# ideafisher/ssUnet-GAN

Measured on AMD Instinct MI355X. Metric: train images/sec (512^2 tiles), higher is better.
Workload: dtype f32; 1 GPU; UNet_R_SS_v2 generator + SRGAN-style discriminator, one G+D step (train_seg_gan.py:182-233), 16 x 3x512x512 tiles per GPU, fp32, Adam lr 2e-5; global_batch=16, tile=512, parallelism=dp1, dead_d_param_grads_of_g_step=computed

## Files before the change

ssunet-gan_amd/csrc/conv_wgrad4.hip:

```cpp
#include "common.h"
#include "conv_thin.h"

namespace {

struct W4Args {
  const float* wide; const float* thin; float* ws;
  int Cw, ldw, ldt, N, H, W, Cout, Cin;
  int groups, nz;
  long long units_per_z;
  int segs_per_row;
};

constexpr int SEG = 32;
constexpr int U = 8;

template <bool THIN_COUT, int KS>
__global__ __launch_bounds__(256) void wgrad4_kernel(const W4Args a) {
  constexpr int R = KS / 2, NT = KS * KS, COLS = U + KS - 1;
  const int lane = threadIdx.x & 63;
  const int wave = threadIdx.x >> 6;
  const int zb = blockIdx.x / a.groups, cg = blockIdx.x - zb * a.groups;
  const int z = zb * 4 + wave;
  const int j = lane & 3;
  const int cw = cg * 64 + lane;
  const bool cw_ok = cw < a.Cw;
  const float* tapT = THIN_COUT ? a.wide : a.thin;
  const float* fixT = THIN_COUT ? a.thin : a.wide;
  const unsigned ldtap = THIN_COUT ? a.ldw : a.ldt, ldfix = THIN_COUT ? a.ldt : a.ldw;
  const unsigned npix = (unsigned)(a.N * a.H * a.W);
  const auto tap_rs = __builtin_amdgcn_make_buffer_rsrc(const_cast<float*>(tapT), 0, (int)(npix * ldtap * 4u), 0x00020000);
  const auto fix_rs = __builtin_amdgcn_make_buffer_rsrc(const_cast<float*>(fixT), 0, (int)(npix * ldfix * 4u), 0x00020000);
  const unsigned chtap = THIN_COUT ? cw : j, chfix = THIN_COUT ? j : cw;
  const bool tap_lane_ok = THIN_COUT ? cw_ok : true, fix_lane_ok = THIN_COUT ? true : cw_ok;
  constexpr unsigned OOB = 0xffffffffu;

  f32x4 acc[NT];
#pragma unroll
  for (int t = 0; t < NT; ++t) acc[t] = f32x4{0.f, 0.f, 0.f, 0.f};

  const int u0 = z * (int)a.units_per_z;
  const int total_units = a.N * a.H * a.segs_per_row;
  int u1 = u0 + (int)a.units_per_z; if (u1 > total_units) u1 = total_units;
  for (int u = u0; u < u1; ++u) {
    const int r = u / a.segs_per_row; const int seg = u - r * a.segs_per_row;
    const int y = r % a.H, n = r / a.H;
    const int x0 = seg * SEG;
    const int x1 = x0 + SEG < a.W ? x0 + SEG : a.W;
    unsigned rowoff[KS]; bool rowok[KS];
#pragma unroll
    for (int q = 0; q < KS; ++q) {
      const int iy = y + q - R;
      rowok[q] = tap_lane_ok && (unsigned)iy < (unsigned)a.H;
      rowoff[q] = ((unsigned)((n * a.H + iy) * a.W) * ldtap + chtap) * 4u;
    }
    const unsigned fixoff = ((unsigned)((n * a.H + y) * a.W) * ldfix + chfix) * 4u;
    for (int xb = x0; xb < x1; xb += U) {
      float f[U], v[KS][COLS];
#pragma unroll
      for (int k = 0; k < U; ++k) {
        const bool ok = fix_lane_ok && (xb + k < x1);
        f[k] = __builtin_bit_cast(float, __builtin_amdgcn_raw_buffer_load_b32(
            fix_rs, ok ? fixoff + (unsigned)(xb + k) * ldfix * 4u : OOB, 0, 0));
      }
#pragma unroll
      for (int c = 0; c < COLS; ++c) {
        const int ix = xb + c - R;
        const bool cok = (unsigned)ix < (unsigned)a.W;
        const unsigned xo = (unsigned)ix * ldtap * 4u;
#pragma unroll
        for (int q = 0; q < KS; ++q)
          v[q][c] = __builtin_bit_cast(float, __builtin_amdgcn_raw_buffer_load_b32(
              tap_rs, (cok && rowok[q]) ? rowoff[q] + xo : OOB, 0, 0));
      }
#pragma unroll
      for (int k = 0; k < U; ++k)
#pragma unroll
        for (int q = 0; q < KS; ++q)
#pragma unroll
          for (int e = 0; e < KS; ++e) {
            if (THIN_COUT) acc[q * KS + e] = __builtin_amdgcn_mfma_f32_4x4x1f32(v[q][k + e], f[k], acc[q * KS + e], 0, 0, 0);
            else acc[q * KS + e] = __builtin_amdgcn_mfma_f32_4x4x1f32(f[k], v[q][k + e], acc[q * KS + e], 0, 0, 0);
          }
    }
  }
  __shared__ float red[4][NT * 4][64];
#pragma unroll
  for (int t = 0; t < NT; ++t)
#pragma unroll
    for (int i = 0; i < 4; ++i) red[wave][t * 4 + i][lane] = acc[t][i];
  __syncthreads();
  float* slab = a.ws + (size_t)zb * NT * a.Cin * a.Cout;
  const int b4 = (lane >> 2) * 4;
  for (int e = wave; e < NT * 4; e += 4) {
    const int t = e >> 2, i = e & 3;
    const float sum = ((red[0][e][lane] + red[1][e][lane]) + red[2][e][lane]) + red[3][e][lane];
    int co, c;
    if (THIN_COUT) { co = j; c = cg * 64 + b4 + i; }
    else { co = cg * 64 + b4 + i; c = j; }
    if (co < a.Cout && c < a.Cin) slab[((size_t)t * a.Cin + c) * a.Cout + co] = sum;
  }
}

__global__ __launch_bounds__(256) void wgrad32_cin_kernel(const W4Args a) {
  const int lane = threadIdx.x & 63, l31 = lane & 31, h = lane >> 5;
  const int wave = threadIdx.x >> 6;
  const int zb = blockIdx.x / a.groups, cg = blockIdx.x - zb * a.groups;
  const int z = zb * 4 + wave;
  const unsigned npix = (unsigned)(a.N * a.H * a.W);
  const auto do_rs = __builtin_amdgcn_make_buffer_rsrc(const_cast<float*>(a.wide), 0, (int)(npix * (unsigned)a.ldw * 4u), 0x00020000);
  const auto in_rs = __builtin_amdgcn_make_buffer_rsrc(const_cast<float*>(a.thin), 0, (int)(npix * (unsigned)a.ldt * 4u), 0x00020000);
  constexpr unsigned OOB = 0xffffffffu;
  const unsigned ldwb = (unsigned)a.ldw * 4u, ldtb = (unsigned)a.ldt * 4u;
  unsigned aoff[2];
#pragma unroll
  for (int f = 0; f < 2; ++f) { const int co = cg * 64 + f * 32 + l31; aoff[f] = co < a.Cout ? (unsigned)co * 4u : OOB; }
  const int t0 = l31 >> 2, c = l31 & 3;
  const int dy0 = t0 / 3 - 1, dx0 = t0 % 3 - 1;
  const bool has1 = l31 < 4;

  f32x16 acc[2][2];
#pragma unroll
  for (int f = 0; f < 2; ++f)
#pragma unroll
    for (int g = 0; g < 2; ++g)
#pragma unroll
      for (int q = 0; q < 16; ++q) acc[f][g][q] = 0.f;

  const int u0 = z * (int)a.units_per_z;
  const int total_units = a.N * a.H * a.segs_per_row;
  int u1 = u0 + (int)a.units_per_z; if (u1 > total_units) u1 = total_units;
  constexpr int UP = 8;
  for (int u = u0; u < u1; ++u) {
    const int r = u / a.segs_per_row; const int seg = u - r * a.segs_per_row;
    const int y = r % a.H, n = r / a.H;
    const int x0 = seg * SEG;
    const int x1 = x0 + SEG < a.W ? x0 + SEG : a.W;
    const unsigned rowpix = (unsigned)((n * a.H + y) * a.W);
    const bool r0ok = (unsigned)(y + dy0) < (unsigned)a.H, r1ok = has1 && y + 1 < a.H;
    const unsigned b0row = (rowpix + (unsigned)(dy0 * a.W)) * ldtb + (unsigned)c * 4u;
    const unsigned b1row = (rowpix + (unsigned)a.W) * ldtb + (unsigned)c * 4u;
    for (int xb = x0; xb < x1; xb += 2 * UP) {
      float av[2][UP], bv[2][UP];
#pragma unroll
      for (int k = 0; k < UP; ++k) {
        const int x = xb + 2 * k + h;
        const bool pok = x < x1;
        const unsigned po = (rowpix + (unsigned)x) * ldwb;
#pragma unroll
        for (int f = 0; f < 2; ++f)
          av[f][k] = __builtin_bit_cast(float, __builtin_amdgcn_raw_buffer_load_b32(do_rs, (pok && aoff[f] != OOB) ? po + aoff[f] : OOB, 0, 0));
        const int ix0 = x + dx0, ix1 = x + 1;
        bv[0][k] = __builtin_bit_cast(float, __builtin_amdgcn_raw_buffer_load_b32(
            in_rs, (pok && r0ok && (unsigned)ix0 < (unsigned)a.W) ? b0row + (unsigned)ix0 * ldtb : OOB, 0, 0));
        bv[1][k] = __builtin_bit_cast(float, __builtin_amdgcn_raw_buffer_load_b32(
            in_rs, (pok && r1ok && ix1 < a.W) ? b1row + (unsigned)ix1 * ldtb : OOB, 0, 0));
      }
#pragma unroll
      for (int k = 0; k < UP; ++k)
#pragma unroll
        for (int f = 0; f < 2; ++f)
#pragma unroll
          for (int g = 0; g < 2; ++g)
            acc[f][g] = __builtin_amdgcn_mfma_f32_32x32x2f32(av[f][k], bv[g][k], acc[f][g], 0, 0, 0);
    }
  }
  __shared__ float red[4][36][64];
#pragma unroll
  for (int f = 0; f < 2; ++f)
#pragma unroll
    for (int g = 0; g < 2; ++g) {
      const int nn = g * 32 + l31;
      if (nn < 36) {
#pragma unroll
        for (int q = 0; q < 16; ++q) red[wave][nn][f * 32 + (q & 3) + 8 * (q >> 2) + 4 * h] = acc[f][g][q];
      }
    }
  __syncthreads();
  float* slab = a.ws + (size_t)zb * 9 * a.Cin * a.Cout;
  for (int e = threadIdx.x; e < 36 * 64; e += 256) {
    const int nn = e >> 6, m = e & 63;
    const float sum = ((red[0][nn][m] + red[1][nn][m]) + red[2][nn][m]) + red[3][nn][m];
    const int co = cg * 64 + m;
    if (co < a.Cout) slab[(size_t)nn * a.Cout + co] = sum;
  }
}

constexpr int TINY_PIX = 4096;

__global__ __launch_bounds__(256) void wgrad_tiny4_kernel(const W4Args a) {
  const int co = threadIdx.x & 7, slot = threadIdx.x >> 3;
  const long long npix = (long long)a.N * a.H * a.W;
  const long long p0 = (long long)blockIdx.x * TINY_PIX;
  const long long p1 = p0 + TINY_PIX < npix ? p0 + TINY_PIX : npix;
  const auto in_rs = __builtin_amdgcn_make_buffer_rsrc(const_cast<float*>(a.thin), 0, (int)((unsigned)npix * (unsigned)a.ldt * 4u), 0x00020000);
  const auto do_rs = __builtin_amdgcn_make_buffer_rsrc(const_cast<float*>(a.wide), 0, (int)((unsigned)npix * (unsigned)a.ldw * 4u), 0x00020000);
  constexpr unsigned OOB = 0xffffffffu;
  const bool co_ok = co < a.Cout;
  f32x4 acc[9];
#pragma unroll
  for (int t = 0; t < 9; ++t) acc[t] = f32x4{0.f, 0.f, 0.f, 0.f};
  for (long long p = p0 + slot; p < p1; p += 32) {
    const int x = (int)(p % a.W); const int y = (int)((p / a.W) % a.H);
    const float g = __builtin_bit_cast(float, __builtin_amdgcn_raw_buffer_load_b32(do_rs, co_ok ? ((unsigned)p * (unsigned)a.ldw + (unsigned)co) * 4u : OOB, 0, 0));
#pragma unroll
    for (int t = 0; t < 9; ++t) {
      const int iy = y + t / 3 - 1, ix = x + t % 3 - 1;
      const bool ok = (unsigned)iy < (unsigned)a.H && (unsigned)ix < (unsigned)a.W;
      const f32x4 v = __builtin_bit_cast(f32x4, __builtin_amdgcn_raw_buffer_load_b128(
          in_rs, ok ? (unsigned)(p + (long long)(t / 3 - 1) * a.W + (t % 3 - 1)) * (unsigned)a.ldt * 4u : OOB, 0, 0));
      acc[t] += v * g;
    }
  }
  __shared__ float red[32][36][8];
#pragma unroll
  for (int t = 0; t < 9; ++t)
#pragma unroll
    for (int c = 0; c < 4; ++c) red[slot][t * 4 + c][co] = acc[t][c];
  __syncthreads();
  float* slab = a.ws + (size_t)blockIdx.x * 9 * a.Cin * a.Cout;
  for (int e = threadIdx.x; e < 36 * 8; e += 256) {
    const int c8 = e & 7, row = e >> 3;
    float sum = 0.f;
#pragma unroll 8
    for (int k = 0; k < 32; ++k) sum += red[k][row][c8];
    const int t = row >> 2, c = row & 3;
    if (c8 < a.Cout && c < a.Cin) slab[((size_t)t * a.Cin + c) * a.Cout + c8] = sum;
  }
}

}

int ssg_wgrad4_kind(const ssg_wgrad_desc* d) {
  if (d->C2 != 0 || d->in_sy != 1 || d->in_sx != 1 || d->GH != d->H || d->GW != d->W) return 0;
  if (d->ntaps == 9) {
    for (int t = 0; t < 9; ++t) if (d->dy[t] != t / 3 - 1 || d->dx[t] != t % 3 - 1) return 0;
  } else if (d->ntaps != 1 || d->dy[0] != 0 || d->dx[0] != 0) {
    return 0;
  }
  if ((long long)d->N * d->H * d->W * (d->ld1 > d->ldd ? d->ld1 : d->ldd) >= (1ll << 30)) return 0;
  if (d->Cout <= 4 && d->C1 >= 16 && d->C1 % 4 == 0) return 5;
  if (d->C1 == 4 && d->Cout <= 8 && d->ntaps == 9) return 7;
  if (d->C1 == 4 && d->ntaps == 9 && d->Cout >= 32 && (long long)d->N * d->H * d->W >= 65536) return 8;
  if (d->C1 == 4) return 6;
  return 0;
}

int ssg_wgrad4_slices(const ssg_wgrad_desc* d, int kind, int* groups, long long* units_per_z, int* segs_per_row) {
  if (kind == 7) {
    if (groups) *groups = 1;
    if (units_per_z) *units_per_z = TINY_PIX;
    if (segs_per_row) *segs_per_row = 1;
    return (int)(((long long)d->N * d->H * d->W + TINY_PIX - 1) / TINY_PIX);
  }
  const int cw = kind == 5 ? d->C1 : d->Cout;
  const int g = (cw + 63) / 64;
  const int spr = (d->W + SEG - 1) / SEG;
  const long long units = (long long)d->N * d->H * spr;
  long long nz = 8192 / g;
  if (nz > units) nz = units;
  if (nz < 1) nz = 1;
  const long long upz = (units + nz - 1) / nz;
  nz = (units + upz - 1) / upz;
  nz = (nz + 3) / 4;
  if (groups) *groups = g;
  if (units_per_z) *units_per_z = upz;
  if (segs_per_row) *segs_per_row = spr;
  return (int)nz;
}

int ssg_wgrad4_launch(const ssg_wgrad_desc* d, int kind, hipStream_t st) {
  W4Args a;
  a.ws = d->ws; a.N = d->N; a.H = d->H; a.W = d->W; a.Cout = d->Cout; a.Cin = d->C1;
  a.nz = ssg_wgrad4_slices(d, kind, &a.groups, &a.units_per_z, &a.segs_per_row);
  const dim3 grid((unsigned)(a.nz * a.groups)), block(256);
  if (kind == 7) {
    a.wide = d->dout; a.Cw = d->Cout; a.ldw = d->ldd; a.thin = d->in1; a.ldt = d->ld1;
    hipLaunchKernelGGL(wgrad_tiny4_kernel, grid, block, 0, st, a);
    SSG_LAUNCH_CHECK();
    return SSG_OK;
  }
  if (kind == 8) {
    a.wide = d->dout; a.Cw = d->Cout; a.ldw = d->ldd; a.thin = d->in1; a.ldt = d->ld1;
    hipLaunchKernelGGL(wgrad32_cin_kernel, grid, block, 0, st, a);
    SSG_LAUNCH_CHECK();
    return SSG_OK;
  }
  if (kind == 5) { a.wide = d->in1; a.Cw = d->C1; a.ldw = d->ld1; a.thin = d->dout; a.ldt = d->ldd; }
  else { a.wide = d->dout; a.Cw = d->Cout; a.ldw = d->ldd; a.thin = d->in1; a.ldt = d->ld1; }
  if (kind == 5 && d->ntaps == 9) hipLaunchKernelGGL((wgrad4_kernel<true, 3>), grid, block, 0, st, a);
  else if (kind == 5) hipLaunchKernelGGL((wgrad4_kernel<true, 1>), grid, block, 0, st, a);
  else if (d->ntaps == 9) hipLaunchKernelGGL((wgrad4_kernel<false, 3>), grid, block, 0, st, a);
  else hipLaunchKernelGGL((wgrad4_kernel<false, 1>), grid, block, 0, st, a);
  SSG_LAUNCH_CHECK();
  return SSG_OK;
}
```

Before: 85.36 images/sec.

## Add row-packed MFMA wgrad kernel for thin-channel 3x3 convolutions

Adds a new weight-gradient kernel that packs (tap, thin-channel) pairs into MFMA rows, so only the real thin channels (up to 3, or Cin_real) times 9 taps fill the 16-row tiles instead of padded channels. Loads are double-buffered in half-segment steps, and padded input channels are written as zeros. It is enabled by default for 3x3 kinds 5, 6 and 8 when the wide tensor is 16-byte aligned, and can be turned off with an env var. The aim is to cut MFMA work and memory traffic wasted on padding in thin-channel layers, at the cost of more per-element scalar loads for the thin operand.

```diff
diff --git a/ssunet-gan_amd/csrc/conv_wgrad4.hip b/ssunet-gan_amd/csrc/conv_wgrad4.hip
--- a/ssunet-gan_amd/csrc/conv_wgrad4.hip
+++ b/ssunet-gan_amd/csrc/conv_wgrad4.hip
@@ -9,6 +9,7 @@
   int groups, nz;
   long long units_per_z;
   int segs_per_row;
+  int ncr;
 };
 
 constexpr int SEG = 32;
@@ -185,6 +186,121 @@
   }
 }
 
+template <bool THIN_COUT, int MT>
+__global__ __launch_bounds__(256) void wgrad_rows_kernel(const W4Args a) {
+  constexpr int ROWS = MT * 16 < 36 ? MT * 16 : 36;
+  constexpr int GH = SEG / 8;
+  const int lane = threadIdx.x & 63, n16 = lane & 15, k = lane >> 4;
+  const int wave = __builtin_amdgcn_readfirstlane(threadIdx.x >> 6);
+  const int zb = blockIdx.x / a.groups, cg = blockIdx.x - zb * a.groups;
+  const int z = zb * 4 + wave;
+  const int NC = THIN_COUT ? a.Cout : a.ncr;
+  const unsigned npix = (unsigned)(a.N * a.H * a.W);
+  const auto w_rs = __builtin_amdgcn_make_buffer_rsrc(const_cast<float*>(a.wide), 0, (int)(npix * (unsigned)a.ldw * 4u), 0x00020000);
+  const auto t_rs = __builtin_amdgcn_make_buffer_rsrc(const_cast<float*>(a.thin), 0, (int)(npix * (unsigned)a.ldt * 4u), 0x00020000);
+  constexpr unsigned OOB = 0xffffffffu;
+  const unsigned ldwb = (unsigned)a.ldw * 4u, ldtb = (unsigned)a.ldt * 4u;
+  const int cq = cg * 64 + 4 * n16;
+  const unsigned boff = cq < a.Cw ? (unsigned)cq * 4u : OOB;
+  int ady[MT], adx[MT]; unsigned aoff[MT]; bool arow[MT];
+#pragma unroll
+  for (int t = 0; t < MT; ++t) {
+    const int m = 16 * t + n16;
+    const int tap = m / NC, ch = m - tap * NC;
+    arow[t] = tap < 9;
+    ady[t] = THIN_COUT ? 1 - tap / 3 : tap / 3 - 1;
+    adx[t] = THIN_COUT ? 1 - tap % 3 : tap % 3 - 1;
+    aoff[t] = (unsigned)(ady[t] * a.W + adx[t]) * ldtb + (unsigned)ch * 4u;
+  }
+
+  f32x4 acc[MT][4];
+#pragma unroll
+  for (int t = 0; t < MT; ++t)
+#pragma unroll
+    for (int j = 0; j < 4; ++j) acc[t][j] = f32x4{0.f, 0.f, 0.f, 0.f};
+
+  const int u0 = z * (int)a.units_per_z;
+  const int total_units = a.N * a.H * a.segs_per_row;
+  int u1 = u0 + (int)a.units_per_z; if (u1 > total_units) u1 = total_units;
+  f32x4 bq[2][GH]; float av[2][MT][GH];
+  int seg, y, n, half = 0;
+  { const int r = u0 / a.segs_per_row; seg = u0 - r * a.segs_per_row; y = r % a.H; n = r / a.H; }
+  const unsigned bvo = (unsigned)k * ldwb + boff;
+  unsigned avo[MT]; int axk[MT];
+#pragma unroll
+  for (int t = 0; t < MT; ++t) { avo[t] = (unsigned)k * ldtb + aoff[t]; axk[t] = k + adx[t]; }
+  auto load = [&](const int s, const bool live) {
+    const int xh = seg * SEG + (SEG / 2) * half;
+    const int x1 = seg * SEG + SEG < a.W ? seg * SEG + SEG : a.W;
+    const int rem = live ? x1 - xh : 0;
+    const unsigned pix0 = (unsigned)((n * a.H + y) * a.W + xh);
+    bool arok[MT];
+#pragma unroll
+    for (int t = 0; t < MT; ++t) arok[t] = arow[t] && (unsigned)(y + ady[t]) < (unsigned)a.H;
+#pragma unroll
+    for (int gi = 0; gi < GH; ++gi) {
+      const bool pok = 4 * gi + k < rem;
+      const unsigned sb = (pix0 + 4u * gi) * ldwb, sa = (pix0 + 4u * gi) * ldtb;
+      const unsigned bo = sb + bvo;
+      bq[s][gi] = __builtin_bit_cast(f32x4, __builtin_amdgcn_raw_buffer_load_b128(w_rs, (pok && boff != OOB) ? bo : OOB, 0, 0));
+#pragma unroll
+      for (int t = 0; t < MT; ++t) {
+        const unsigned ao = sa + avo[t];
+        const bool ok = pok && arok[t] && (unsigned)(xh + 4 * gi + axk[t]) < (unsigned)a.W;
+        av[s][t][gi] = __builtin_bit_cast(float, __builtin_amdgcn_raw_buffer_load_b32(t_rs, ok ? ao : OOB, 0, 0));
+      }
+    }
+    if (half) { if (++seg == a.segs_per_row) { seg = 0; if (++y == a.H) { y = 0; ++n; } } }
+    half ^= 1;
+  };
+  auto mma = [&](const int s) {
+#pragma unroll
+    for (int gi = 0; gi < GH; ++gi)
+#pragma unroll
+      for (int t = 0; t < MT; ++t)
+#pragma unroll
+        for (int j = 0; j < 4; ++j) acc[t][j] = __builtin_amdgcn_mfma_f32_16x16x4f32(av[s][t][gi], bq[s][gi][j], acc[t][j], 0, 0, 0);
+  };
+  if (u0 < u1) {
+    load(0, true);
+    for (int u = u0; u < u1; ++u) {
+      load(1, true);
+      mma(0);
+      load(0, u + 1 < u1);
+      mma(1);
+    }
+  }
+  __shared__ float red[4][ROWS][64];
+#pragma unroll
+  for (int t = 0; t < MT; ++t)
+#pragma unroll
+    for (int r = 0; r < 4; ++r) {
+      const int m = 16 * t + 4 * k + r;
+      if (m < ROWS) *(f32x4*)&red[wave][m][4 * n16] = f32x4{acc[t][0][r], acc[t][1][r], acc[t][2][r], acc[t][3][r]};
+    }
+  __syncthreads();
+  float* slab = a.ws + (size_t)zb * 9 * a.Cin * a.Cout;
+  const int live = 9 * NC;
+  for (int e = threadIdx.x; e < ROWS * 64; e += 256) {
+    const int m = e >> 6, cc = e & 63;
+    const float sum = ((red[0][m][cc] + red[1][m][cc]) + red[2][m][cc]) + red[3][m][cc];
+    const int tap = m / NC, ch = m - tap * NC;
+    const int cw = cg * 64 + cc;
+    if (m < live && cw < a.Cw) {
+      if (THIN_COUT) slab[((size_t)tap * a.Cin + cw) * a.Cout + ch] = sum;
+      else slab[((size_t)tap * a.Cin + ch) * a.Cout + cw] = sum;
+    }
+  }
+  if (!THIN_COUT) {
+    const int npad = a.Cin - NC;
+    for (int e = threadIdx.x; e < 9 * npad * 64; e += 256) {
+      const int r = e >> 6, cw = cg * 64 + (e & 63);
+      const int tap = r / npad, ch = NC + r - tap * npad;
+      if (cw < a.Cw) slab[((size_t)tap * a.Cin + ch) * a.Cout + cw] = 0.f;
+    }
+  }
+}
+
 constexpr int TINY_PIX = 4096;
 
 __global__ __launch_bounds__(256) void wgrad_tiny4_kernel(const W4Args a) {
@@ -268,8 +384,18 @@
   return (int)nz;
 }
 
+static bool rows_form(const ssg_wgrad_desc* d, int kind) {
+  if (d->ntaps != 9 || (kind != 5 && kind != 6 && kind != 8)) return false;
+  const char* e = getenv("SSG_WGRAD_ROWS");
+  if (e && atoi(e) == 0) return false;
+  const float* wide = kind == 5 ? d->in1 : d->dout;
+  const int ldw = kind == 5 ? d->ld1 : d->ldd;
+  return ((uintptr_t)wide & 15) == 0 && ldw % 4 == 0;
+}
+
 int ssg_wgrad4_launch(const ssg_wgrad_desc* d, int kind, hipStream_t st) {
   W4Args a;
+  a.ncr = 0;
   a.ws = d->ws; a.N = d->N; a.H = d->H; a.W = d->W; a.Cout = d->Cout; a.Cin = d->C1;
   a.nz = ssg_wgrad4_slices(d, kind, &a.groups, &a.units_per_z, &a.segs_per_row);
   const dim3 grid((unsigned)(a.nz * a.groups)), block(256);
@@ -279,6 +405,22 @@
     SSG_LAUNCH_CHECK();
     return SSG_OK;
   }
+  if (rows_form(d, kind)) {
+    if (kind == 5) {
+      a.wide = d->in1; a.Cw = d->C1; a.ldw = d->ld1; a.thin = d->dout; a.ldt = d->ldd;
+      if (d->Cout <= 1) hipLaunchKernelGGL((wgrad_rows_kernel<true, 1>), grid, block, 0, st, a);
+      else if (d->Cout <= 3) hipLaunchKernelGGL((wgrad_rows_kernel<true, 2>), grid, block, 0, st, a);
+      else hipLaunchKernelGGL((wgrad_rows_kernel<true, 3>), grid, block, 0, st, a);
+    } else {
+      a.wide = d->dout; a.Cw = d->Cout; a.ldw = d->ldd; a.thin = d->in1; a.ldt = d->ld1;
+      a.ncr = d->Cin_real >= 1 && d->Cin_real < 4 ? d->Cin_real : 4;
+      if (a.ncr <= 1) hipLaunchKernelGGL((wgrad_rows_kernel<false, 1>), grid, block, 0, st, a);
+      else if (a.ncr <= 3) hipLaunchKernelGGL((wgrad_rows_kernel<false, 2>), grid, block, 0, st, a);
+      else hipLaunchKernelGGL((wgrad_rows_kernel<false, 3>), grid, block, 0, st, a);
+    }
+    SSG_LAUNCH_CHECK();
+    return SSG_OK;
+  }
   if (kind == 8) {
     a.wide = d->dout; a.Cw = d->Cout; a.ldw = d->ldd; a.thin = d->in1; a.ldt = d->ld1;
     hipLaunchKernelGGL(wgrad32_cin_kernel, grid, block, 0, st, a);
```

Result: faster. 86.24 images/sec, median of 6 (+1.0%).
